# bkj/pytorch-graphsage

Measured on AMD Instinct MI355X. Metric: seed-nodes/sec, higher is better.
Workload: dtype bf16; 1 GPU; Reddit-shaped mean-aggregator 2-layer fanout 25/10 hidden 128/128 (BASELINE configs[1]); N=232965 D=602 nnz=98191232; batch_per_gpu=512, global_batch=512, rng=philox, engine=fused, launch=cmdlist, pipelined=False, batch_queue=True, parallelism=dp1, ranks=1

## Files before the change

include/gsage.h:

```cpp
#ifndef GSAGE_H
#define GSAGE_H

#include <stdint.h>

#ifdef __cplusplus
extern "C" {
#endif

#define GSAGE_ABI_VERSION 6

enum { GSAGE_F32 = 0, GSAGE_BF16 = 1, GSAGE_FP8 = 2 };
enum {
    GSAGE_OK = 0,
    GSAGE_EINVAL = -1,
    GSAGE_ELAUNCH = -2,
    GSAGE_ENODEV = -3
};
enum { GSAGE_POOL_MAX = 0, GSAGE_POOL_MEAN = 1 };
enum { GSAGE_ACT_NONE = 0, GSAGE_ACT_RELU = 1, GSAGE_ACT_TANH = 2 };

int gsage_abi_version(void);
const char *gsage_last_error(void);
uint64_t gsage_launch_count(void);
int gsage_debug_abort_trace(int fd);
// ... 83 lines not shown
int gsage_mt_choice_device(uint32_t *state, int64_t high, int64_t count, int32_t *out, void *stream);
int gsage_mt_choice_segments(uint32_t *state, int64_t high, int64_t n_seg, const int64_t *seg_off,
                             const int64_t *seg_cnt, int32_t *out, void *stream);

int gsage_mt_choice_par(uint32_t *state, int64_t high, int64_t n_seg, const int64_t *seg_cum, const int64_t *seg_off,
                        int64_t n_total, int32_t *out, const uint64_t *table, void *scratch, int64_t scratch_bytes,
                        int32_t n_wg, int32_t units_per_wg, void *stream);
int64_t gsage_mt_choice_par_scratch(int32_t n_wg);
int gsage_mt_jump_table(uint64_t *out, int64_t words);
int64_t gsage_mt_jump_table_words(void);
int gsage_mt_jump_host(const uint32_t *state, const uint64_t *poly, uint32_t *out);
void gsage_mt_permutation(void *mt, int64_t n, int64_t *out);

int gsage_gather_mean(const void *table, int dtype, int64_t ld, const int64_t *ids, int64_t M,
                      int32_t n, int64_t D, void *out, int out_dtype, int64_t out_ld,
                      void *stream);

int gsage_gather_mean_multi(int32_t n_seg, const void *const *tables, const int64_t *const *ids,
                            void *const *outs, const int64_t *M, const int32_t *n, int dtype,
                            int64_t ld, int64_t D, int out_dtype, int64_t out_ld, void *stream);

int gsage_quantize_fp8(const void *table, int dtype, int64_t ld, int64_t n_rows, int64_t D, void *table_q,
                       int64_t ld_q, float *scale, void *stream);

int gsage_gather_rows_fp8(const void *table_q, int64_t ld, const float *scale, const int64_t *ids, int64_t M,
                          int64_t D, void *out, int out_dtype, int64_t out_ld, void *stream);

int gsage_gather_mean_fp8(const void *table_q, int64_t ld, const float *scale, const int64_t *ids, int64_t M,
                          int32_t n, int64_t D, void *out, int out_dtype, int64_t out_ld, void *stream);
int gsage_gather_mean_multi_fp8(int32_t n_seg, const void *const *tables_q, const int64_t *const *ids,
                                void *const *outs, const int64_t *M, const int32_t *n, const float *scale,
                                int64_t ld, int64_t D, int out_dtype, int64_t out_ld, void *stream);

int gsage_segment_mean_bwd(const float *dagg, int64_t ld, int64_t M, int32_t n, int64_t D,
                           float *dneibs, int64_t out_ld, void *stream);

int gsage_scatter_add_rows(const float *rows, int64_t ld, const int64_t *ids, int64_t M,
                           int32_t n, int64_t D, float scale, float *table_grad,
                           int64_t table_ld, void *stream);

int gsage_linear_nt(const void *A, int dtype, int64_t lda, const int64_t *a_rows,
                    int a_rows_group0_only, const void *W, int64_t ldw, const float *bias,
                    void *C, int c_dtype, int64_t ldc, int64_t M, int64_t N, int64_t K, int act,
                    int groups, int64_t a_gstride, int64_t w_gstride, int64_t c_gstride,
                    void *stream);

int64_t gsage_packed_weight_elems(int64_t N, int64_t K, int32_t groups);
int gsage_pack_weight(const void *W, int dtype, int64_t ldw, int64_t w_gstride, int64_t N, int64_t K,
                      int32_t groups, void *Wp, void *stream);
int gsage_linear_nt_packed(const void *A, int64_t lda, const int64_t *a_rows, int a_rows_group0_only,
                           const void *Wp, const float *bias, void *C, int c_dtype, int64_t ldc,
                           int64_t M, int64_t N, int64_t K, int act, int groups, int64_t a_gstride,
                           int64_t c_gstride, void *stream);

int gsage_wgrad(const void *dC, int dtype, int64_t ldc, const void *A, int64_t lda, int64_t a_gstride, int64_t M,
                int64_t Ntot, int64_t K,
                int64_t n_per_group, int64_t rows_per_split, float *slabs, int64_t ldk, float *out,
                int64_t out_gstride, void *stream);
int gsage_wgrad_slabs(int64_t M, int64_t rows_per_split);
typedef struct gsage_wgrad_desc {
    const void *dC;
    const void *A;
    float *slabs;
    int64_t ldc, lda, a_gstride;
    int64_t M, Ntot, K, n_per_group, ldk, rows_per_split;
    const int64_t *a_rows;
} gsage_wgrad_desc;
int gsage_wgrad_multi(int32_t n_prob, const gsage_wgrad_desc *probs, int dtype, void *stream);
int gsage_wgrad_pair_ok(int dtype, int64_t M, int64_t Ntot, int64_t n_per_group, int64_t rows_per_split);
int gsage_wgrad_ticks_next(int64_t *tick, int64_t *tick1, int64_t inc1, int64_t *tick2, int64_t inc2);

int gsage_pool_mlp(const void *A, int dtype, int64_t lda, const int64_t *a_rows, const void *W,
                   int64_t ldw, const float *bias, int64_t M, int32_t n, int64_t H, int64_t K,
                   int pool, float *pooled, int64_t pooled_ld, int32_t *argmax, void *pooled_bf16,
                   int64_t pooled_bf16_ld, uint32_t *relu_mask, void *stream);

int gsage_pool_mlp_packed(const void *A, int64_t lda, const int64_t *a_rows, const void *Wp,
                          const float *bias, int64_t M, int32_t n, int64_t H, int64_t K, int pool,
                          float *pooled, int64_t pooled_ld, int32_t *argmax, void *pooled_bf16,
                          int64_t pooled_bf16_ld, uint32_t *relu_mask, void *stream);

int gsage_pool_route_bwd(const float *g, int64_t ldg, const float *pooled, int64_t ldp,
                         const int32_t *argmax, int64_t lda, int64_t M, int32_t n, int32_t H, void *out,
                         int out_dtype, int64_t ldo, void *stream);

int gsage_pool_route_mean_bwd(const float *g, int64_t ldg, const uint32_t *relu_mask, int64_t M, int32_t n,
                              int32_t H, void *out, int out_dtype, int64_t ldo, float *bias_part, int32_t n_part,
                              void *stream);

int gsage_pool_bias_partials(const float *g, int64_t ldg, const float *pooled, int64_t ldp, int64_t M,
                             int32_t H, float *part, int32_t n_part, void *stream);

int gsage_pool_merge_bwd(const void *Hprev, int dtype, int64_t ldh, const float *DX, int64_t ldx, int64_t r_x,
                         const float *DN, int64_t ldn, int64_t r0, void *dH, int64_t ldo, int64_t R,
                         int32_t D, void *stream);

int gsage_attn_aggregate(const float *na, int64_t na_ld, const float *xa, int64_t xa_ld,
                         const void *table, int dtype, int64_t ld, const int64_t *ids, int64_t M,
                         int32_t n, int64_t Ha, int64_t D, float *agg, int64_t agg_ld, float *ws,
                         void *stream);
int gsage_attn_aggregate_lp(const float *na, int64_t na_ld, const float *xa, int64_t xa_ld, const void *table,
                            int dtype, int64_t ld, const int64_t *ids, int64_t M, int32_t n, int64_t Ha, int64_t D,
                            float *agg, int64_t agg_ld, float *ws, void *agg_lp, int64_t agg_lp_ld, void *stream);
int gsage_attn_mlp2_fwd(const void *hid, int dtype, int64_t ldh, const void *W2, int64_t ldw, float *a, int64_t lda,
                        int64_t M, int32_t Ha, void *stream);
int gsage_attn_mlp2_bwd(const float *dan, int64_t ldn, const float *dax, int64_t ldx, const void *hid, int dtype,
// ... 249 lines not shown
```

pytorch-graphsage_amd/_native.py:

```python
import ctypes
import os

_HERE = os.path.dirname(os.path.abspath(__file__))
LIB_PATH = os.path.join(_HERE, "libgsage_hip.so")

F32, BF16, FP8 = 0, 1, 2
POOL_MAX, POOL_MEAN = 0, 1
ACT_NONE, ACT_RELU, ACT_TANH = 0, 1, 2
SEG_MEAN, SEG_MAX, SEG_SOFTMAX_WEIGHTED, SEG_WEIGHTED_MEAN = 0, 1, 2, 3
ABI_VERSION = 6

_vp = ctypes.c_void_p
_i64 = ctypes.c_int64
_i32 = ctypes.c_int32
_u32 = ctypes.c_uint32
_u64 = ctypes.c_uint64
_int = ctypes.c_int
_f32 = ctypes.c_float

SIGNATURES = {
    "gsage_abi_version": (_int, []),
    "gsage_last_error": (ctypes.c_char_p, []),
    "gsage_launch_count": (_u64, []),
    "gsage_debug_abort_trace": (_int, [_int]),
# ... 13 lines not shown
    "gsage_cmdlist_side_begin": (_int, []),
    "gsage_cmdlist_side_end": (_int, []),
    "gsage_cmdlist_join": (_int, []),
    "gsage_cmdlist_destroy": (None, [_vp]),
    "gsage_host_call": (_int, [_vp, _vp, _vp]),
    "gsage_comm_load": (_int, [ctypes.c_char_p]),
    "gsage_comm_unique_id": (_int, [_vp]),
    "gsage_comm_create": (_int, [_vp, _i32, _i32, ctypes.POINTER(_vp)]),
    "gsage_comm_destroy": (_int, [_vp]),
    "gsage_comm_all_reduce_f32": (_int, [_vp, _vp, _i64, _i32, _vp]),
    "gsage_comm_all_gather": (_int, [_vp, _vp, _vp, _i64, _vp]),
    "gsage_comm_group": (_int, [_vp, _i32, _vp]),
    "gsage_sort_rows_temp_bytes": (_i64, [_i64, _i32]),
    "gsage_sort_rows": (_int, [_vp, _i64, _i64, _i64, _i32, _vp, _vp, _vp, _i64, _vp]),
    "gsage_segment_sum_rows": (_int, [_vp, _vp, _i64, _vp, _i64, _i64, _vp, _i64, _i32, _f32, _vp, _i64, _vp]),
    "gsage_head_l1_sharded": (_int, [_vp, _i64, _vp, _vp, _vp, _i64, _i64, _i64, _vp, _vp, _int, _i64, _vp, _vp]),
    "gsage_sample_csr_sel": (_int, [_vp, _vp, _i64, _vp, _i64, _i32, _vp, _vp, _vp, _vp]),
    "gsage_sample_dense": (_int, [_vp, _i64, _i64, _vp, _i64, _vp, _i32, _vp, _vp, _vp]),
    "gsage_sample_csr_philox": (_int, [_vp, _vp, _i64, _vp, _i64, _i32, _u32, _u64, _vp, _u64, _u64,
                                       _vp, _vp, _vp, _vp]),
    "gsage_sample_hops_philox": (_int, [_vp, _vp, _i64, _vp, _i64, _i32, _vp, _u32, _u64, _vp, _u64, _u64,
                                        _vp, _vp, _i64, _vp, _vp]),
    "gsage_sample_hops": (_int, [_vp, _vp]),
    "gsage_counter_add": (_int, [_vp, _u64, _vp]),
    "gsage_copy_pair": (_int, [_vp, _vp, _i64, _vp, _vp, _i64, _vp]),
    "gsage_mt_create": (_vp, [_u32]),
    "gsage_mt_destroy": (None, [_vp]),
    "gsage_mt_seed": (None, [_vp, _u32]),
    "gsage_mt_choice_i32": (_i64, [_vp, _i64, _i64, _vp]),
    "gsage_mt_permutation": (None, [_vp, _i64, _vp]),
    "gsage_mt_choice_device": (_int, [_vp, _i64, _i64, _vp, _vp]),
    "gsage_mt_choice_segments": (_int, [_vp, _i64, _i64, _vp, _vp, _vp, _vp]),
    "gsage_mt_choice_par": (_int, [_vp, _i64, _i64, _vp, _vp, _i64, _vp, _vp, _vp, _i64, _i32, _i32, _vp]),
    "gsage_mt_choice_par_scratch": (_i64, [_i32]),
    "gsage_mt_jump_table": (_int, [_vp, _i64]),
    "gsage_mt_jump_table_words": (_i64, []),
    "gsage_mt_jump_host": (_int, [_vp, _vp, _vp]),
    "gsage_head_n_valid_next": (_int, [_vp]),
    "gsage_gather_role_next": (_int, [_vp]),
    "gsage_hops_role_next": (_int, [_vp]),
    "gsage_gather_mean": (_int, [_vp, _int, _i64, _vp, _i64, _i32, _i64, _vp, _int, _i64, _vp]),
    "gsage_gather_mean_multi": (_int, [_i32, _vp, _vp, _vp, _vp, _vp, _int, _i64, _i64, _int, _i64, _vp]),
    "gsage_gather_mean_multi_adam": (_int, [_i32, _vp, _vp, _vp, _vp, _vp, _int, _i64, _i64, _int, _i64,
                                            _vp, _vp, _vp]),
    "gsage_quantize_fp8": (_int, [_vp, _int, _i64, _i64, _i64, _vp, _i64, _vp, _vp]),
    "gsage_gather_rows_fp8": (_int, [_vp, _i64, _vp, _vp, _i64, _i64, _vp, _int, _i64, _vp]),
    "gsage_gather_mean_fp8": (_int, [_vp, _i64, _vp, _vp, _i64, _i32, _i64, _vp, _int, _i64, _vp]),
    "gsage_gather_mean_multi_fp8": (_int, [_i32, _vp, _vp, _vp, _vp, _vp, _vp, _i64, _i64, _int, _i64, _vp]),
    "gsage_segment_mean_bwd": (_int, [_vp, _i64, _i64, _i32, _i64, _vp, _i64, _vp]),
    "gsage_scatter_add_rows": (_int, [_vp, _i64, _vp, _i64, _i32, _i64, _f32, _vp, _i64, _vp]),
    "gsage_linear_nt": (_int, [_vp, _int, _i64, _vp, _int, _vp, _i64, _vp, _vp, _int, _i64, _i64,
                               _i64, _i64, _int, _int, _i64, _i64, _i64, _vp]),
    "gsage_packed_weight_elems": (_i64, [_i64, _i64, _i32]),
    "gsage_pack_weight": (_int, [_vp, _int, _i64, _i64, _i64, _i64, _i32, _vp, _vp]),
    "gsage_linear_nt_packed": (_int, [_vp, _i64, _vp, _int, _vp, _vp, _vp, _int, _i64, _i64, _i64, _i64, _int,
                                      _int, _i64, _i64, _vp]),
    "gsage_wgrad": (_int, [_vp, _int, _i64, _vp, _i64, _i64, _i64, _i64, _i64, _i64, _i64, _vp, _i64, _vp,
                           _i64, _vp]),
    "gsage_wgrad_slabs": (_int, [_i64, _i64]),
    "gsage_pool_route_bwd": (_int, [_vp, _i64, _vp, _i64, _vp, _i64, _i64, _i32, _i32, _vp, _int, _i64, _vp]),
    "gsage_wgrad_multi": (_int, [_i32, _vp, _int, _vp]),
    "gsage_wgrad_pair_ok": (_int, [_int, _i64, _i64, _i64, _i64]),
    "gsage_wgrad_ticks_next": (_int, [_vp, _vp, _i64, _vp, _i64]),
    "gsage_clip_adam_meet": (_int, [_vp, _vp]),
    "gsage_gather_adam_capacity": (_int, [_int, _i64]),
    "gsage_head_ce": (_int, [_vp, _i64, _vp, _vp, _vp, _i32, _i32, _i32, _vp, _vp, _int, _i64, _vp, _vp,
                             _vp, _vp, _vp, _i64, _vp]),
    "gsage_head_ce_scratch": (_i64, [_i32, _i32, _i32]),
    "gsage_mean_tail_ce": (_int, [_vp, _i32, _i32, _vp, _i64, _vp, _i64, _vp, _vp, _i32, _vp, _vp, _i64,
                                  _vp, _vp, _vp, _vp, _vp, _vp, _int, _vp]),
    "gsage_mean_tail_ce_scratch": (_i64, [_i32, _i32]),
    "gsage_mean_tail_mfma": (_int, [_vp, _i32, _i32, _vp, _i64, _vp, _i64, _vp, _vp, _i32, _vp, _vp, _i64,
                                    _vp, _vp, _vp, _vp, _vp, _vp, _vp]),
    "gsage_mean_tail_mfma_scratch": (_i64, [_i32, _i32]),
    "gsage_mean_tail_mfma_sampler_wgs": (_i32, [_i64, _i64]),
    "gsage_clip_adam_step": (_int, [_vp, _vp, _vp, _vp, _i64, _vp, _vp, _vp, _f32, _f32, _f32, _f32,
                                    _f32, _vp, _int, _i32, _vp, _i32, _vp, _i64, _vp, _i64, _vp]),
    "gsage_finalize_grads": (_int, [_vp, _i32, _i64, _vp, _vp, _vp, _vp, _i64, _vp, _i64, _vp]),
    "gsage_finalize_partials": (_int, [_i32, _i64]),
    "gsage_grad_sqnorm": (_int, [_vp, _i64, _vp, _i32, _vp]),
    "gsage_zero_rows": (_int, [_vp, _i64, _vp, _i64, _i64, _vp]),
    "gsage_colsum_partials": (_int, [_vp, _i64, _i64, _i32, _vp, _i32, _vp]),
    "gsage_rows_catch_up": (_int, [_vp, _vp, _i64, _vp, _i64, _i32, _vp]),
    "gsage_rows_catch_up_all": (_int, [_vp, _i32, _vp]),
    "gsage_rows_sqnorm": (_int, [_vp, _vp, _i64, _vp, _i64, _i32, _vp, _i32, _vp]),
    "gsage_rows_adam": (_int, [_vp, _vp, _i64, _vp, _i64, _i32, _vp, _i32, _vp]),
    "gsage_adam_partials": (_int, [_i64]),
    "gsage_prep_weights": (_int, [_vp, _i32, _i64, _vp, _i64, _vp, _i64, _vp]),
    "gsage_bwd_merge": (_int, [_vp, _int, _i64, _vp, _i64, _i64, _vp, _i64, _i64, _i64, _i32, _i32, _vp,
                               _vp, _vp]),
    "gsage_pool_mlp": (_int, [_vp, _int, _i64, _vp, _vp, _i64, _vp, _i64, _i32, _i64, _i64, _int,
                              _vp, _i64, _vp, _vp, _i64, _vp, _vp]),
    "gsage_pool_mlp_packed": (_int, [_vp, _i64, _vp, _vp, _vp, _i64, _i32, _i64, _i64, _int, _vp, _i64, _vp, _vp,
                                     _i64, _vp, _vp]),
    "gsage_pool_route_mean_bwd": (_int, [_vp, _i64, _vp, _i64, _i32, _i32, _vp, _int, _i64, _vp, _i32, _vp]),
    "gsage_pool_bias_partials": (_int, [_vp, _i64, _vp, _i64, _i64, _i32, _vp, _i32, _vp]),
    "gsage_pool_merge_bwd": (_int, [_vp, _int, _i64, _vp, _i64, _i64, _vp, _i64, _i64, _vp, _i64, _i64, _i32, _vp]),
    "gsage_attn_aggregate": (_int, [_vp, _i64, _vp, _i64, _vp, _int, _i64, _vp, _i64, _i32, _i64,
                                    _i64, _vp, _i64, _vp, _vp]),
    "gsage_attn_aggregate_lp": (_int, [_vp, _i64, _vp, _i64, _vp, _int, _i64, _vp, _i64, _i32, _i64,
                                       _i64, _vp, _i64, _vp, _vp, _i64, _vp]),
    "gsage_attn_fused_ok": (_int, [_int, _i64, _i64, _i32, _i64]),
    "gsage_attn_fused_fwd": (_int, [_vp, _int, _i64, _vp, _i64, _vp, _i64, _vp, _i64, _vp, _i64, _i64, _i32, _i64, _vp,
                                    _i64, _vp, _i64, _vp, _vp, _i64, _vp]),
    "gsage_attn_fused_bwd": (_int, [_vp, _int, _i64, _vp, _i64, _vp, _i64, _vp, _i64, _vp, _vp, _i64, _vp, _i64, _vp, _i64,
                                    _i64, _i32, _i64, _vp, _i64, _vp, _i64, _vp, _i64, _vp]),
# ... 253 lines not shown
```

pytorch-graphsage_amd/csrc/gsage_packed.hip:

```cpp
#include "gsage_common.h"
#include "gsage_gather_dev.h"
#include "gsage_mma_dev.h"
#include "gsage_sample_dev.h"

namespace gsage {

#ifndef GSAGE_WP_R
#define GSAGE_WP_R 4
#endif
constexpr int WP_R = GSAGE_WP_R;
constexpr int WP_WAIT = ((6 * (WP_R - 1)) & 15) | (7 << 4) | (15 << 8) | (((6 * (WP_R - 1)) >> 4) << 14);
static_assert(WP_R == 4 || WP_R == 6 || WP_R == 8, "WP_R");
static_assert(WP_R != 4 || WP_WAIT == 0x4F72, "vmcnt(18)");
constexpr int WP_NBUF = WP_R + 1;
constexpr int WP_UNROLL = 24;

struct PackedParams {
    const uint16_t *A;
    const uint16_t *Wp;
    const float *bias;
    const int64_t *a_rows;
    void *C;
    int64_t lda, ldc;
    int64_t M, N, K;
    int64_t a_gstride, wp_gstride, c_gstride;
    int32_t kc_total;
    int32_t a_rows_group0_only;
    int32_t c_dtype;
};

constexpr int WP_SMEM_VEC = (BM * (BN + 4) * 4) / 16 > WP_NBUF * (BM * CH) ? (BM * (BN + 4) * 4) / 16 : WP_NBUF * (BM * CH);

template <int ACT, int GN, bool HOPS>
__global__ void __launch_bounds__(256)
k_linear_nt_packed(const PackedParams p, const TailGather tg, const HopsParams hp)
{
    constexpr int EPC = 8;
    constexpr int ATILE = BM * CH;
    __shared__ vec16 smem[WP_SMEM_VEC];
    if (HOPS && blockIdx.z + 1 == gridDim.z) {
        sample_hops_workgroup<false>(hp, (int)(blockIdx.y * gridDim.x + blockIdx.x), reinterpret_cast<int64_t *>(smem));
        return;
    }
    if (GN > 0 && blockIdx.z + 1 == gridDim.z) {
        gather_role<(GN > 0 ? GN : 1), 2>(tg, (int)(blockIdx.y * gridDim.x + blockIdx.x));
        return;
    }

    const int tid = threadIdx.x;
    const int lane = tid & 63;
    const int wave = tid >> 6;
    const int g = blockIdx.z;
    const int64_t m0 = (int64_t)blockIdx.x * BM;
    const int64_t n0 = (int64_t)blockIdx.y * BN;
    const uint16_t *A = p.A + (int64_t)g * p.a_gstride;
    const int64_t *a_rows = (p.a_rows && (g == 0 || !p.a_rows_group0_only)) ? p.a_rows : nullptr;
    const int nk = (int)((p.K + 63) / 64);
    const int64_t jb_last = (p.N - 1) >> 5;
    const int64_t jb = min((n0 >> 5) + wave, jb_last);
    const vec16 *wp = reinterpret_cast<const vec16 *>(p.Wp + (int64_t)g * p.wp_gstride) +
                      (jb * p.kc_total) * 64 + lane;

    const int cdst = lane & 7;
    const uint16_t *a_src[2];
#pragma unroll
    for (int s2 = 0; s2 < 2; ++s2) {
        const int R = 32 * s2 + 8 * wave + (lane >> 3);
        const int row = (R & ~9) | ((R & 1) << 3) | ((R >> 3) & 1);
        int64_t m = m0 + row;
        if (m >= p.M) m = p.M - 1;
        const int64_t r = a_rows ? a_rows[m] : m;
        a_src[s2] = A + r * p.lda + (cdst ^ (row & 7)) * EPC;
    }
    const int a_dst0 = (8 * wave) * CH, a_dst1 = (32 + 8 * wave) * CH;

    vec16 wr[WP_R][4];
    auto issue_tile = [&](int kt, int buf, vec16 (&w)[4]) {
        vec16 *base = smem + buf * ATILE;
        const int64_t ko = (int64_t)kt * 64;
        __builtin_amdgcn_sched_barrier(0);
        __builtin_amdgcn_global_load_lds((global_void_t *)(a_src[0] + ko), (lds_void_t *)(base + a_dst0), 16, 0, 0);
        __builtin_amdgcn_global_load_lds((global_void_t *)(a_src[1] + ko), (lds_void_t *)(base + a_dst1), 16, 0, 0);
#pragma unroll
        for (int kk = 0; kk < 4; ++kk) w[kk] = wp[(int64_t)(kt * 4 + kk) * 64];
        __builtin_amdgcn_sched_barrier(0);
    };

    f32x16_t acc0, acc1;
#pragma unroll
    for (int r = 0; r < 16; ++r) { acc0[r] = 0.f; acc1[r] = 0.f; }
    const int arow0 = lane & 31, arow1 = arow0 + 32;

    auto compute_tile = [&](int kt, const vec16 (&w)[4]) {
        const vec16 *sA = smem + (kt % WP_NBUF) * ATILE;
        vec16 fa0[4], fa1[4];
#pragma unroll
        for (int kk = 0; kk < 4; ++kk) {
            const int ch = kk * 2 + (lane >> 5);
            fa0[kk] = sA[lds_slot(arow0, ch)];
            fa1[kk] = sA[lds_slot(arow1, ch)];
        }
        __builtin_amdgcn_s_waitcnt(0xC07F);
        __builtin_amdgcn_sched_barrier(0);
#pragma unroll
        for (int kk = 0; kk < 4; ++kk) {
            mma_chunk<uint16_t>::run(fa0[kk], w[kk], acc0);
            mma_chunk<uint16_t>::run(fa1[kk], w[kk], acc1);
        }
        __builtin_amdgcn_sched_barrier(0);
    };

    int kt = 0, phase = 0;
    if (nk > WP_R) {
#pragma unroll
        for (int t = 0; t < WP_R; ++t) issue_tile(t, t, wr[t]);
#pragma unroll
        for (int u = 0; u < WP_UNROLL; ++u) {
            if (kt + WP_R >= nk) { phase = u % WP_R; goto drain; }
            __builtin_amdgcn_s_waitcnt(WP_WAIT);
            __builtin_amdgcn_s_barrier();
            compute_tile(kt, wr[u % WP_R]);
            issue_tile(kt + WP_R, (kt + WP_R) % WP_NBUF, wr[u % WP_R]);
            ++kt;
        }
        for (;;) {
#pragma unroll
            for (int s = 0; s < WP_R; ++s) {
                if (kt + WP_R >= nk) { phase = s; goto drain; }
                __builtin_amdgcn_s_waitcnt(WP_WAIT);
                __builtin_amdgcn_s_barrier();
                compute_tile(kt, wr[s]);
                issue_tile(kt + WP_R, (kt + WP_R) % WP_NBUF, wr[s]);
                ++kt;
            }
        }
    } else {
#pragma unroll
        for (int t = 0; t < WP_R; ++t)
            if (t < nk) issue_tile(t, t, wr[t]);
    }
drain:
    __builtin_amdgcn_s_waitcnt(0x0F70);
    __builtin_amdgcn_s_barrier();
#pragma unroll
    for (int t = 0; t < WP_R; ++t) {
        if (kt + t < nk) {
            const int idx = (phase + t) % WP_R;
#pragma unroll
            for (int s = 0; s < WP_R; ++s)
                if (idx == s) compute_tile(kt + t, wr[s]);
        }
    }

    const float *bias = p.bias ? p.bias + (int64_t)g * p.N : nullptr;
    const int esz = p.c_dtype == GSAGE_BF16 ? 2 : 4;
    const int epc = 16 / esz;
    const int64_t cbase = (int64_t)g * p.c_gstride + n0;
    const bool wide = n0 + BN <= p.N && p.ldc % epc == 0 && cbase % epc == 0 && ((uintptr_t)p.C % 16) == 0;
    const int jl = wave * 32 + (lane & 31);
    const float bj = (bias && n0 + jl < p.N) ? bias[n0 + jl] : 0.f;
    if (wide) {
        __syncthreads();
        const int ldt = BN + epc;
#pragma unroll
        for (int rb = 0; rb < 2; ++rb) {
            const f32x16_t &acc = rb ? acc1 : acc0;
#pragma unroll
            for (int r = 0; r < 16; ++r) {
                const int i = rb * 32 + (r & 3) + 8 * (r >> 2) + 4 * (lane >> 5);
                const float v = apply_act(acc[r] + bj, ACT);
                if (p.c_dtype == GSAGE_BF16)
                    ((uint16_t *)smem)[i * ldt + jl] = f32_to_bf16(v);
                else
                    ((float *)smem)[i * ldt + jl] = v;
            }
        }
        __syncthreads();
        const int cpr = BN / epc;
        for (int q = tid; q < BM * cpr; q += 256) {
            const int row = q / cpr, ch = q - row * cpr;
            const int64_t m = m0 + row;
            if (m < p.M) {
                const vec16 v = *reinterpret_cast<const vec16 *>((const char *)smem +
                                                                 ((size_t)row * ldt + ch * epc) * esz);
                *reinterpret_cast<vec16 *>((char *)p.C + ((size_t)m * p.ldc + cbase + ch * epc) * esz) = v;
            }
        }
        return;
    }
    const int64_t j = n0 + jl;
#pragma unroll
    for (int rb = 0; rb < 2; ++rb) {
        const f32x16_t &acc = rb ? acc1 : acc0;
#pragma unroll
        for (int r = 0; r < 16; ++r) {
            const int64_t m = m0 + rb * 32 + (r & 3) + 8 * (r >> 2) + 4 * (lane >> 5);
            if (m < p.M && j < p.N) {
                const float v = apply_act(acc[r] + bj, ACT);
                const int64_t off = m * p.ldc + (int64_t)g * p.c_gstride + j;
                if (p.c_dtype == GSAGE_BF16)
                    ((uint16_t *)p.C)[off] = f32_to_bf16(v);
                else
                    ((float *)p.C)[off] = v;
            }
        }
    }
}

constexpr int WS_TPW = 8;
constexpr int WS_LDT = BN + 8;

template <int NK> constexpr int ws_ring() { return NK == 3 ? 3 : 4; }
template <int NK> constexpr size_t ws_lds_bytes()
{
    return (size_t)(ws_ring<NK>() + 1) * BM * CH * 16 + (size_t)BM * WS_LDT * 2 + (size_t)WS_TPW * 2 * 256 * 4;
}

template <int N>
__device__ __forceinline__ void ws_wait_vm()
{
    static_assert(N >= 0 && N < 64, "vmcnt is six bits");
    asm volatile("s_waitcnt vmcnt(%0)" ::"n"(N) : "memory");
}

template <int BASE, int STEP>
__device__ __forceinline__ void ws_wait_vm_sel(int t)
{
    if (t == 0) ws_wait_vm<BASE>();
    else if (t == 1) ws_wait_vm<BASE + STEP>();
    else if (t == 2) ws_wait_vm<BASE + 2 * STEP>();
    else ws_wait_vm<BASE + 3 * STEP>();
}

template <int ACT, int NK>
__global__ void __launch_bounds__(256)
k_linear_nt_packed_ws(const PackedParams p, const int tpw)
{
    constexpr int R = ws_ring<NK>(), TR = R / NK, NBUF = R + 1, ATILE = BM * CH, NST = 4;
    constexpr int STEADY = 2 * (R - 1) + NST * TR;
    extern __shared__ __attribute__((aligned(16))) char ws_smem[];
    vec16 *ring = reinterpret_cast<vec16 *>(ws_smem);
    uint16_t *stage = reinterpret_cast<uint16_t *>(ws_smem + (size_t)NBUF * ATILE * 16);
    uint32_t *rid_s = reinterpret_cast<uint32_t *>(ws_smem + (size_t)NBUF * ATILE * 16 + (size_t)BM * WS_LDT * 2);

    const int tid = threadIdx.x, lane = tid & 63;
    const int wave = __builtin_amdgcn_readfirstlane(tid >> 6);
    const int g = blockIdx.z;
    const int64_t n0 = (int64_t)blockIdx.y * BN;
    const int64_t n_tiles = (p.M + BM - 1) / BM;
    const int64_t tile0 = (int64_t)blockIdx.x * tpw;
    const uint16_t *A = p.A + (int64_t)g * p.a_gstride;
// ... 389 lines not shown
                sum += v;
                if (v > best) { best = v; arg = r; }
            }
            if (p.pool_mode == GSAGE_POOL_MAX) {
                p.pooled[seg * p.pooled_ld + j] = best;
                if (p.pooled_b) p.pooled_b[seg * p.pooled_b_ld + j] = f32_to_bf16(best);
                if (p.argmax) p.argmax[seg * p.N + j] = arg;
            } else {
                p.pooled[seg * p.pooled_ld + j] = sum / (float)p.pool_n;
                if (p.pooled_b) p.pooled_b[seg * p.pooled_b_ld + j] = f32_to_bf16(sum / (float)p.pool_n);
            }
        }
    }
}


template <typename TW>
__global__ void __launch_bounds__(256)
k_pack_weight(const TW *__restrict__ W, int64_t ldw, int64_t w_gstride, int64_t N, int64_t K,
              int32_t kc_total, int32_t jb_total, int32_t groups, uint16_t *__restrict__ Wp)
{
    const int64_t total = (int64_t)groups * jb_total * kc_total * 64;
    const int64_t stride = (int64_t)gridDim.x * 256;
    for (int64_t t = (int64_t)blockIdx.x * 256 + threadIdx.x; t < total; t += stride) {
        const int lane = (int)(t & 63);
        int64_t u = t >> 6;
        const int kc = (int)(u % kc_total);
        u /= kc_total;
        const int jb = (int)(u % jb_total);
        const int g = (int)(u / jb_total);
        const int64_t j = (int64_t)jb * 32 + (lane & 31);
        const int64_t k0 = (int64_t)kc * 16 + (lane >> 5) * 8;
        uint16_t out[8];
#pragma unroll
        for (int e = 0; e < 8; ++e) {
            float v = 0.f;
            if (j < N && k0 + e < K) {
                const TW w = W[(int64_t)g * w_gstride + j * ldw + k0 + e];
                v = sizeof(TW) == 2 ? bf16_to_f32((uint16_t)w) : (float)w;
            }
            out[e] = f32_to_bf16(v);
        }
        vec16 o;
#pragma unroll
        for (int e = 0; e < 4; ++e) o[e] = (uint32_t)out[2 * e] | ((uint32_t)out[2 * e + 1] << 16);
        reinterpret_cast<vec16 *>(Wp)[t] = o;
    }
}

}

using namespace gsage;

extern "C" {

int64_t gsage_packed_weight_elems(int64_t N, int64_t K, int32_t groups)
{
    return (int64_t)groups * ceil_div(N, 32) * (ceil_div(K, 64) * 4) * 64 * 8;
}

int gsage_pack_weight(const void *W, int dtype, int64_t ldw, int64_t w_gstride, int64_t N, int64_t K,
                      int32_t groups, void *Wp, void *stream)
{
    GSAGE_REQUIRE(W && Wp && N > 0 && K > 0 && groups >= 1 && ldw >= K, "pack_weight: bad arguments");
    GSAGE_REQUIRE(dtype == GSAGE_BF16 || dtype == GSAGE_F32, "pack_weight: bad dtype %d", dtype);
    GSAGE_REQUIRE(((uintptr_t)Wp % 16) == 0, "pack_weight: output must be 16-byte aligned");
    const int32_t kc = (int32_t)(ceil_div(K, 64) * 4), jb = (int32_t)ceil_div(N, 32);
    const int64_t slots = (int64_t)groups * jb * kc * 64;
    int64_t blocks = ceil_div(slots, 256);
    if (blocks > 4096) blocks = 4096;
    if (dtype == GSAGE_BF16)
        launch(k_pack_weight<uint16_t>, dim3((unsigned)blocks), dim3(256), 0, (hipStream_t)stream,
               (const uint16_t *)W, ldw, w_gstride, N, K, kc, jb, groups, (uint16_t *)Wp);
    else
        launch(k_pack_weight<float>, dim3((unsigned)blocks), dim3(256), 0, (hipStream_t)stream,
               (const float *)W, ldw, w_gstride, N, K, kc, jb, groups, (uint16_t *)Wp);
    return check_launch("pack_weight");
}

int gsage_linear_nt_packed(const void *A, int64_t lda, const int64_t *a_rows, int a_rows_group0_only,
                           const void *Wp, const float *bias, void *C, int c_dtype, int64_t ldc,
                           int64_t M, int64_t N, int64_t K, int act, int groups, int64_t a_gstride,
                           int64_t c_gstride, void *stream)
{
    const gsage_tail_gather_desc *gd = take_gather_role();
    const gsage_hops_desc *hd = t_hops_role;
    t_hops_role = nullptr;
    GSAGE_REQUIRE(A && Wp && C, "linear_nt_packed: null pointer");
    GSAGE_REQUIRE(M >= 0 && N > 0 && K > 0, "linear_nt_packed: bad sizes");
    GSAGE_REQUIRE(c_dtype == GSAGE_BF16 || c_dtype == GSAGE_F32, "linear_nt_packed: bad c_dtype");
    GSAGE_REQUIRE(groups >= 1 && groups <= 65535, "linear_nt_packed: bad group count");
    GSAGE_REQUIRE(act >= ACT_NONE && act <= ACT_TANH, "linear_nt_packed: bad activation code");
    GSAGE_REQUIRE(lda % 64 == 0 && ceil_div(K, 64) * 64 <= lda && ((uintptr_t)A % 16) == 0 &&
                  ((uintptr_t)Wp % 16) == 0, "linear_nt_packed: A rows must be whole zero-padded 128-byte lines");
    if (M == 0) return GSAGE_OK;
    PackedParams p;
    p.A = (const uint16_t *)A; p.Wp = (const uint16_t *)Wp; p.bias = bias; p.a_rows = a_rows; p.C = C;
    p.lda = lda; p.ldc = ldc; p.M = M; p.N = N; p.K = K;
    p.a_gstride = a_gstride; p.c_gstride = c_gstride;
    p.kc_total = (int32_t)(ceil_div(K, 64) * 4);
    p.wp_gstride = ceil_div(N, 32) * (int64_t)p.kc_total * 64 * 8;
    p.a_rows_group0_only = a_rows_group0_only; p.c_dtype = c_dtype;
    dim3 grid((unsigned)ceil_div(M, BM), (unsigned)ceil_div(N, BN), (unsigned)groups);
    hipStream_t s = (hipStream_t)stream;
    TailGather tg = {};
    HopsParams hp = {};
    if (hd) {
        GSAGE_REQUIRE(!(gd && gd->rows > 0) && act == ACT_RELU && !hd->dense_adj,
                      "linear_nt_packed: the sampler role rides with the ReLU projection, walks a CSR, and excludes the "
                      "gather role");
        size_t lds = 0;
        const int rc = fill_hops(hp, lds, *hd);
        if (rc != GSAGE_OK) return rc;
        const int64_t slots = (int64_t)grid.x * grid.y;
        hp.spw = (int32_t)ceil_div(hd->B > 0 ? hd->B : 1, slots);
        int64_t widest = 1, width = 1;
        for (int k = 1; k <= hp.n_hops; ++k) { width *= hp.fan[k]; widest = width > widest ? width : widest; }
        GSAGE_REQUIRE(sizeof(int64_t) * 2 * (size_t)hp.spw * (size_t)widest <= sizeof(vec16) * WP_SMEM_VEC,
                      "linear_nt_packed: the sampler role's frontier (%d seeds x %lld ids, twice) does not fit the "
                      "projection's LDS", hp.spw, (long long)widest);
        grid.z += 1;
        launch(k_linear_nt_packed<ACT_RELU, 0, true>, grid, dim3(256), 0, s, p, tg, hp);
        return check_launch("linear_nt_packed");
    }
    if (gd && gd->rows > 0) {
        const int rc = fill_gather_role(tg, *gd, "linear_nt_packed (gather role)");
        if (rc != GSAGE_OK) return rc;
        GSAGE_REQUIRE(act == ACT_RELU && (gd->n == 10 || gd->n == 5),
                      "linear_nt_packed: the gather role rides with the ReLU projection, fan-out 5 or 10");
        tg.n_wg = (int32_t)(grid.x * grid.y);
        grid.z += 1;
        if (gd->n == 10) launch(k_linear_nt_packed<ACT_RELU, 10, false>, grid, dim3(256), 0, s, p, tg, hp);
        else launch(k_linear_nt_packed<ACT_RELU, 5, false>, grid, dim3(256), 0, s, p, tg, hp);
        return check_launch("linear_nt_packed");
    }
    {
        const char *ws_env = getenv("GSAGE_K5_WS");
        const bool ws_on = !ws_env || atoi(ws_env) != 0;
        const int nk = (int)ceil_div(K, 64);
        const int tr = nk == 1 ? 4 : nk == 2 ? 2 : 1;
        const int64_t n_tiles = ceil_div(M, BM);
        if (ws_on && c_dtype == GSAGE_BF16 && nk <= 4 && N % BN == 0 && ldc % 8 == 0 && c_gstride % 8 == 0 &&
            ((uintptr_t)C % 16) == 0 && n_tiles >= 4 * tr && (act == ACT_RELU || act == ACT_NONE)) {
            int dev = 0, cus = 256;
            if (hipGetDevice(&dev) == hipSuccess) {
                int v = 0;
                if (hipDeviceGetAttribute(&v, hipDeviceAttributeMultiprocessorCount, dev) == hipSuccess && v > 0) cus = v;
                else (void)hipGetLastError();
            } else (void)hipGetLastError();
            const int64_t slices = (int64_t)grid.y * groups;
            int64_t per = ceil_div(2 * (int64_t)cus, slices);
            if (per < 1) per = 1;
            int64_t tpw = ceil_div(n_tiles, per);
            if (const char *e = getenv("GSAGE_K5_WS_TPW")) tpw = atoi(e);
            if (tpw < tr) tpw = tr;
            if (tpw > WS_TPW) tpw = WS_TPW;
            grid.x = (unsigned)ceil_div(n_tiles, tpw);
#define GSAGE_WS_LAUNCH(ACTV, NKV)                                                                                        \
            do {                                                                                                      \
                static bool raised = false;                                                                           \
                if (!raised) {                                                                                        \
                    if (hipFuncSetAttribute((const void *)k_linear_nt_packed_ws<ACTV, NKV>,                           \
                                            hipFuncAttributeMaxDynamicSharedMemorySize, (int)ws_lds_bytes<NKV>()) != hipSuccess) { \
                        (void)hipGetLastError();                                                                      \
                        set_error("linear_nt_packed: cannot raise the dynamic LDS limit");                          \
                        return GSAGE_ELAUNCH;                                                                         \
                    }                                                                                                 \
                    raised = true;                                                                                    \
                }                                                                                                     \
                launch(k_linear_nt_packed_ws<ACTV, NKV>, grid, dim3(256), ws_lds_bytes<NKV>(), s, p, (int)tpw);       \
            } while (0)
#define GSAGE_WS_NK(ACTV)                                                                                                 \
            do {                                                                                                      \
                if (nk == 1) GSAGE_WS_LAUNCH(ACTV, 1);                                                                \
                else if (nk == 2) GSAGE_WS_LAUNCH(ACTV, 2);                                                           \
                else if (nk == 3) GSAGE_WS_LAUNCH(ACTV, 3);                                                           \
                else GSAGE_WS_LAUNCH(ACTV, 4);                                                                        \
            } while (0)
            if (act == ACT_RELU) GSAGE_WS_NK(ACT_RELU);
            else GSAGE_WS_NK(ACT_NONE);
#undef GSAGE_WS_NK
#undef GSAGE_WS_LAUNCH
            return check_launch("linear_nt_packed");
        }
    }
    if (act == ACT_RELU)
        launch(k_linear_nt_packed<ACT_RELU, 0, false>, grid, dim3(256), 0, s, p, tg, hp);
    else if (act == ACT_TANH)
        launch(k_linear_nt_packed<ACT_TANH, 0, false>, grid, dim3(256), 0, s, p, tg, hp);
    else
        launch(k_linear_nt_packed<ACT_NONE, 0, false>, grid, dim3(256), 0, s, p, tg, hp);
    return check_launch("linear_nt_packed");
}

int gsage_pool_mlp_packed(const void *A, int64_t lda, const int64_t *a_rows, const void *Wp,
                          const float *bias, int64_t M, int32_t n, int64_t H, int64_t K, int pool,
                          float *pooled, int64_t pooled_ld, int32_t *argmax, void *pooled_bf16,
                          int64_t pooled_bf16_ld, uint32_t *relu_mask, void *stream)
{
    GSAGE_REQUIRE(A && Wp && pooled && pooled_ld >= H, "pool_mlp_packed: bad pointers / output");
    GSAGE_REQUIRE(M >= 0 && H > 0 && K > 0, "pool_mlp_packed: bad sizes");
    GSAGE_REQUIRE(n >= 1 && n <= BM, "pool_mlp_packed: fanout must be in [1, %d]", BM);
    GSAGE_REQUIRE(!relu_mask || H % 32 == 0, "pool_mlp_packed: relu_mask needs H % 32 == 0");
    GSAGE_REQUIRE(!pooled_bf16 || pooled_bf16_ld >= H, "pool_mlp_packed: bad bf16 output");
    GSAGE_REQUIRE(pool == GSAGE_POOL_MAX || pool == GSAGE_POOL_MEAN, "pool_mlp_packed: bad pool mode");
    GSAGE_REQUIRE(lda % 64 == 0 && ceil_div(K, 64) * 64 <= lda && ((uintptr_t)A % 16) == 0 &&
                  ((uintptr_t)Wp % 16) == 0, "pool_mlp_packed: A rows must be whole zero-padded 128-byte lines");
    if (M == 0) return GSAGE_OK;
    PoolPackedParams p;
    p.A = (const uint16_t *)A; p.Wp = (const uint16_t *)Wp; p.bias = bias; p.a_rows = a_rows; p.lda = lda;
    p.M = M * (int64_t)n; p.N = H; p.K = K; p.kc_total = (int32_t)(ceil_div(K, 64) * 4);
    p.pool_n = n; p.pool_groups = BM / n; p.pool_mode = pool; p.pooled = pooled; p.pooled_ld = pooled_ld;
    p.pooled_b = (uint16_t *)pooled_bf16; p.pooled_b_ld = pooled_bf16_ld; p.argmax = argmax;
    p.relu_mask = relu_mask;
    const int64_t subs = ceil_div(M, p.pool_groups);
    dim3 grid((unsigned)subs, (unsigned)ceil_div(H, 256), 1);
    static const bool regs = [] { const char *e = getenv("GSAGE_POOL_REGS"); return !e || atoi(e) != 0; }();
    const bool rp = regs && pool == GSAGE_POOL_MAX && !relu_mask;
    hipStream_t s = (hipStream_t)stream;
    if (rp && n == 10) launch(k_pool_mlp_packed<4, 10>, grid, dim3(256), 0, s, p);
    else if (rp && n == 25) launch(k_pool_mlp_packed<4, 25>, grid, dim3(256), 0, s, p);
    else if (rp && n == 5) launch(k_pool_mlp_packed<4, 5>, grid, dim3(256), 0, s, p);
    else if (rp && n == 15) launch(k_pool_mlp_packed<4, 15>, grid, dim3(256), 0, s, p);
    else if (rp && n == 20) launch(k_pool_mlp_packed<4, 20>, grid, dim3(256), 0, s, p);
    else launch(k_pool_mlp_packed<4, 0>, grid, dim3(256), 0, s, p);
    return check_launch("pool_mlp_packed");
}

}
```

Measured before the change: 6.368 million seed-nodes/sec.

## Add tall 128-row tile variant to packed projection kernel when grid oversubscribes CUs

```diff
diff --git a/include/gsage.h b/include/gsage.h
--- a/include/gsage.h
+++ b/include/gsage.h
@@ -159,6 +159,7 @@
                            const void *Wp, const float *bias, void *C, int c_dtype, int64_t ldc,
                            int64_t M, int64_t N, int64_t K, int act, int groups, int64_t a_gstride,
                            int64_t c_gstride, void *stream);
+int gsage_packed_last_rows(void);
 
 int gsage_wgrad(const void *dC, int dtype, int64_t ldc, const void *A, int64_t lda, int64_t a_gstride, int64_t M,
                 int64_t Ntot, int64_t K,
diff --git a/pytorch-graphsage_amd/_native.py b/pytorch-graphsage_amd/_native.py
--- a/pytorch-graphsage_amd/_native.py
+++ b/pytorch-graphsage_amd/_native.py
@@ -89,6 +89,7 @@
     "gsage_linear_nt": (_int, [_vp, _int, _i64, _vp, _int, _vp, _i64, _vp, _vp, _int, _i64, _i64,
                                _i64, _i64, _int, _int, _i64, _i64, _i64, _vp]),
     "gsage_packed_weight_elems": (_i64, [_i64, _i64, _i32]),
+    "gsage_packed_last_rows": (_int, []),
     "gsage_pack_weight": (_int, [_vp, _int, _i64, _i64, _i64, _i64, _i32, _vp, _vp]),
     "gsage_linear_nt_packed": (_int, [_vp, _i64, _vp, _int, _vp, _vp, _vp, _int, _i64, _i64, _i64, _i64, _int,
                                       _int, _i64, _i64, _vp]),
diff --git a/pytorch-graphsage_amd/csrc/gsage_packed.hip b/pytorch-graphsage_amd/csrc/gsage_packed.hip
--- a/pytorch-graphsage_amd/csrc/gsage_packed.hip
+++ b/pytorch-graphsage_amd/csrc/gsage_packed.hip
@@ -8,11 +8,23 @@
 #ifndef GSAGE_WP_R
 #define GSAGE_WP_R 4
 #endif
+#ifndef GSAGE_WP_RT
+#define GSAGE_WP_RT 4
+#endif
 constexpr int WP_R = GSAGE_WP_R;
-constexpr int WP_WAIT = ((6 * (WP_R - 1)) & 15) | (7 << 4) | (15 << 8) | (((6 * (WP_R - 1)) >> 4) << 14);
+constexpr int WP_BMT = 128;
+constexpr int WP_RT = GSAGE_WP_RT;
+constexpr int wp_tile_vm(int bmt) { return bmt / 32 + 4; }
+constexpr int wp_wait(int bmt, int r)
+{
+    return ((wp_tile_vm(bmt) * (r - 1)) & 15) | (7 << 4) | (15 << 8) | (((wp_tile_vm(bmt) * (r - 1)) >> 4) << 14);
+}
 static_assert(WP_R == 4 || WP_R == 6 || WP_R == 8, "WP_R");
-static_assert(WP_R != 4 || WP_WAIT == 0x4F72, "vmcnt(18)");
-constexpr int WP_NBUF = WP_R + 1;
+static_assert(WP_RT == 4 || WP_RT == 6, "WP_RT");
+static_assert(wp_tile_vm(WP_BMT) * (WP_RT - 1) < 64 && wp_tile_vm(BM) * (WP_R - 1) < 64, "vmcnt is six bits");
+static_assert(WP_R != 4 || wp_wait(BM, WP_R) == 0x4F72, "vmcnt(18)");
+static_assert(wp_wait(WP_BMT, 4) == 0x4F78, "vmcnt(24)");
+static_assert(wp_wait(WP_BMT, 6) == 0x8F78, "vmcnt(40)");
 constexpr int WP_UNROLL = 24;
 
 struct PackedParams {
@@ -29,15 +41,30 @@
     int32_t c_dtype;
 };
 
-constexpr int WP_SMEM_VEC = (BM * (BN + 4) * 4) / 16 > WP_NBUF * (BM * CH) ? (BM * (BN + 4) * 4) / 16 : WP_NBUF * (BM * CH);
-
-template <int ACT, int GN, bool HOPS>
+constexpr int wp_smem_vec(int bmt, int r)
+{
+    return (bmt * (BN + 4) * 4) / 16 > (r + 1) * (bmt * CH) ? (bmt * (BN + 4) * 4) / 16 : (r + 1) * (bmt * CH);
+}
+
+template <int ACT, int GN, bool HOPS, int BMT = BM, int R = WP_R>
 __global__ void __launch_bounds__(256)
 k_linear_nt_packed(const PackedParams p, const TailGather tg, const HopsParams hp)
 {
     constexpr int EPC = 8;
-    constexpr int ATILE = BM * CH;
-    __shared__ vec16 smem[WP_SMEM_VEC];
+    constexpr int NRB = BMT / 32;
+    constexpr int NBUF = R + 1;
+    constexpr int WAIT = wp_wait(BMT, R);
+    constexpr int ATILE = BMT * CH;
+    static_assert(BMT == BM || BMT == WP_BMT, "BMT");
+    static_assert(WP_UNROLL % R == 0, "WP_UNROLL");
+    vec16 *smem;
+    if constexpr (BMT == BM) {
+        __shared__ vec16 smem_static[wp_smem_vec(BMT, R)];
+        smem = smem_static;
+    } else {
+        extern __shared__ __attribute__((aligned(16))) vec16 smem_tall[];
+        smem = smem_tall;
+    }
     if (HOPS && blockIdx.z + 1 == gridDim.z) {
         sample_hops_workgroup<false>(hp, (int)(blockIdx.y * gridDim.x + blockIdx.x), reinterpret_cast<int64_t *>(smem));
         return;
@@ -51,7 +78,7 @@
     const int lane = tid & 63;
     const int wave = tid >> 6;
     const int g = blockIdx.z;
-    const int64_t m0 = (int64_t)blockIdx.x * BM;
+    const int64_t m0 = (int64_t)blockIdx.x * BMT;
     const int64_t n0 = (int64_t)blockIdx.y * BN;
     const uint16_t *A = p.A + (int64_t)g * p.a_gstride;
     const int64_t *a_rows = (p.a_rows && (g == 0 || !p.a_rows_group0_only)) ? p.a_rows : nullptr;
@@ -62,92 +89,96 @@
                       (jb * p.kc_total) * 64 + lane;
 
     const int cdst = lane & 7;
-    const uint16_t *a_src[2];
-#pragma unroll
-    for (int s2 = 0; s2 < 2; ++s2) {
-        const int R = 32 * s2 + 8 * wave + (lane >> 3);
-        const int row = (R & ~9) | ((R & 1) << 3) | ((R >> 3) & 1);
+    const uint16_t *a_src[NRB];
+#pragma unroll
+    for (int s2 = 0; s2 < NRB; ++s2) {
+        const int R0 = 32 * s2 + 8 * wave + (lane >> 3);
+        const int row = (R0 & ~9) | ((R0 & 1) << 3) | ((R0 >> 3) & 1);
         int64_t m = m0 + row;
         if (m >= p.M) m = p.M - 1;
         const int64_t r = a_rows ? a_rows[m] : m;
         a_src[s2] = A + r * p.lda + (cdst ^ (row & 7)) * EPC;
     }
-    const int a_dst0 = (8 * wave) * CH, a_dst1 = (32 + 8 * wave) * CH;
-
-    vec16 wr[WP_R][4];
+    const int a_dst0 = (8 * wave) * CH;
+
+    vec16 wr[R][4];
     auto issue_tile = [&](int kt, int buf, vec16 (&w)[4]) {
         vec16 *base = smem + buf * ATILE;
         const int64_t ko = (int64_t)kt * 64;
         __builtin_amdgcn_sched_barrier(0);
-        __builtin_amdgcn_global_load_lds((global_void_t *)(a_src[0] + ko), (lds_void_t *)(base + a_dst0), 16, 0, 0);
-        __builtin_amdgcn_global_load_lds((global_void_t *)(a_src[1] + ko), (lds_void_t *)(base + a_dst1), 16, 0, 0);
+#pragma unroll
+        for (int s2 = 0; s2 < NRB; ++s2)
+            __builtin_amdgcn_global_load_lds((global_void_t *)(a_src[s2] + ko),
+                                             (lds_void_t *)(base + a_dst0 + s2 * 32 * CH), 16, 0, 0);
 #pragma unroll
         for (int kk = 0; kk < 4; ++kk) w[kk] = wp[(int64_t)(kt * 4 + kk) * 64];
         __builtin_amdgcn_sched_barrier(0);
     };
 
-    f32x16_t acc0, acc1;
-#pragma unroll
-    for (int r = 0; r < 16; ++r) { acc0[r] = 0.f; acc1[r] = 0.f; }
-    const int arow0 = lane & 31, arow1 = arow0 + 32;
+    f32x16_t acc[NRB];
+#pragma unroll
+    for (int rb = 0; rb < NRB; ++rb)
+#pragma unroll
+        for (int r = 0; r < 16; ++r) acc[rb][r] = 0.f;
+    const int arow0 = lane & 31;
 
     auto compute_tile = [&](int kt, const vec16 (&w)[4]) {
-        const vec16 *sA = smem + (kt % WP_NBUF) * ATILE;
-        vec16 fa0[4], fa1[4];
+        const vec16 *sA = smem + (kt % NBUF) * ATILE;
+        vec16 fa[NRB][4];
 #pragma unroll
         for (int kk = 0; kk < 4; ++kk) {
             const int ch = kk * 2 + (lane >> 5);
-            fa0[kk] = sA[lds_slot(arow0, ch)];
-            fa1[kk] = sA[lds_slot(arow1, ch)];
+#pragma unroll
+            for (int rb = 0; rb < NRB; ++rb) fa[rb][kk] = sA[lds_slot(arow0 + 32 * rb, ch)];
         }
         __builtin_amdgcn_s_waitcnt(0xC07F);
         __builtin_amdgcn_sched_barrier(0);
 #pragma unroll
         for (int kk = 0; kk < 4; ++kk) {
-            mma_chunk<uint16_t>::run(fa0[kk], w[kk], acc0);
-            mma_chunk<uint16_t>::run(fa1[kk], w[kk], acc1);
+#pragma unroll
+            for (int rb = 0; rb < NRB; ++rb) mma_chunk<uint16_t>::run(fa[rb][kk], w[kk], acc[rb]);
         }
         __builtin_amdgcn_sched_barrier(0);
     };
 
     int kt = 0, phase = 0;
-    if (nk > WP_R) {
-#pragma unroll
-        for (int t = 0; t < WP_R; ++t) issue_tile(t, t, wr[t]);
+    if (nk > R) {
+#pragma unroll
+        for (int t = 0; t < R; ++t) issue_tile(t, t, wr[t]);
 #pragma unroll
         for (int u = 0; u < WP_UNROLL; ++u) {
-            if (kt + WP_R >= nk) { phase = u % WP_R; goto drain; }
-            __builtin_amdgcn_s_waitcnt(WP_WAIT);
+            if (kt + R >= nk) { phase = u % R; goto drain; }
+            __builtin_amdgcn_s_waitcnt(WAIT);
             __builtin_amdgcn_s_barrier();
-            compute_tile(kt, wr[u % WP_R]);
-            issue_tile(kt + WP_R, (kt + WP_R) % WP_NBUF, wr[u % WP_R]);
+            compute_tile(kt, wr[u % R]);
+            issue_tile(kt + R, (kt + R) % NBUF, wr[u % R]);
             ++kt;
         }
         for (;;) {
 #pragma unroll
-            for (int s = 0; s < WP_R; ++s) {
-                if (kt + WP_R >= nk) { phase = s; goto drain; }
-                __builtin_amdgcn_s_waitcnt(WP_WAIT);
+            for (int s = 0; s < R; ++s) {
+                if (kt + R >= nk) { phase = s; goto drain; }
+                __builtin_amdgcn_s_waitcnt(WAIT);
                 __builtin_amdgcn_s_barrier();
                 compute_tile(kt, wr[s]);
-                issue_tile(kt + WP_R, (kt + WP_R) % WP_NBUF, wr[s]);
+                issue_tile(kt + R, (kt + R) % NBUF, wr[s]);
                 ++kt;
             }
         }
     } else {
 #pragma unroll
-        for (int t = 0; t < WP_R; ++t)
+        for (int t = 0; t < R; ++t)
             if (t < nk) issue_tile(t, t, wr[t]);
     }
 drain:
     __builtin_amdgcn_s_waitcnt(0x0F70);
     __builtin_amdgcn_s_barrier();
 #pragma unroll
-    for (int t = 0; t < WP_R; ++t) {
+    for (int t = 0; t < R; ++t) {
         if (kt + t < nk) {
-            const int idx = (phase + t) % WP_R;
-#pragma unroll
-            for (int s = 0; s < WP_R; ++s)
+            const int idx = (phase + t) % R;
+#pragma unroll
+            for (int s = 0; s < R; ++s)
                 if (idx == s) compute_tile(kt + t, wr[s]);
         }
     }
@@ -163,12 +194,11 @@
         __syncthreads();
         const int ldt = BN + epc;
 #pragma unroll
-        for (int rb = 0; rb < 2; ++rb) {
-            const f32x16_t &acc = rb ? acc1 : acc0;
+        for (int rb = 0; rb < NRB; ++rb) {
 #pragma unroll
             for (int r = 0; r < 16; ++r) {
                 const int i = rb * 32 + (r & 3) + 8 * (r >> 2) + 4 * (lane >> 5);
-                const float v = apply_act(acc[r] + bj, ACT);
+                const float v = apply_act(acc[rb][r] + bj, ACT);
                 if (p.c_dtype == GSAGE_BF16)
                     ((uint16_t *)smem)[i * ldt + jl] = f32_to_bf16(v);
                 else
@@ -177,7 +207,7 @@
         }
         __syncthreads();
         const int cpr = BN / epc;
-        for (int q = tid; q < BM * cpr; q += 256) {
+        for (int q = tid; q < BMT * cpr; q += 256) {
             const int row = q / cpr, ch = q - row * cpr;
             const int64_t m = m0 + row;
             if (m < p.M) {
@@ -190,13 +220,12 @@
     }
     const int64_t j = n0 + jl;
 #pragma unroll
-    for (int rb = 0; rb < 2; ++rb) {
-        const f32x16_t &acc = rb ? acc1 : acc0;
+    for (int rb = 0; rb < NRB; ++rb) {
 #pragma unroll
         for (int r = 0; r < 16; ++r) {
             const int64_t m = m0 + rb * 32 + (r & 3) + 8 * (r >> 2) + 4 * (lane >> 5);
             if (m < p.M && j < p.N) {
-                const float v = apply_act(acc[r] + bj, ACT);
+                const float v = apply_act(acc[rb][r] + bj, ACT);
                 const int64_t off = m * p.ldc + (int64_t)g * p.c_gstride + j;
                 if (p.c_dtype == GSAGE_BF16)
                     ((uint16_t *)p.C)[off] = f32_to_bf16(v);
@@ -692,7 +721,64 @@
 
 using namespace gsage;
 
+namespace {
+
+constexpr size_t WP_TALL_LDS = sizeof(vec16) * wp_smem_vec(WP_BMT, WP_RT);
+constexpr int WP_MAX_DEV = 64;
+
+thread_local int t_last_rows = 0;
+
+int current_cus(int &dev)
+{
+    int cus = 256;
+    dev = 0;
+    if (hipGetDevice(&dev) == hipSuccess) {
+        int v = 0;
+        if (hipDeviceGetAttribute(&v, hipDeviceAttributeMultiprocessorCount, dev) == hipSuccess && v > 0) cus = v;
+        else (void)hipGetLastError();
+    } else (void)hipGetLastError();
+    return cus;
+}
+
+bool wants_tall_tiles(int64_t M, int64_t N, int groups, int cus)
+{
+    const char *e = getenv("GSAGE_K5_BM");
+    const int forced = e ? atoi(e) : 0;
+    if (M < WP_BMT || forced == BM) return false;
+    if (forced == WP_BMT) return true;
+    return ceil_div(M, BM) * ceil_div(N, BN) * groups > cus;
+}
+
+template <int ACT, int GN, bool HOPS>
+bool tall_tiles_ok(int dev)
+{
+    static std::atomic<int> state[WP_MAX_DEV];
+    if (dev < 0 || dev >= WP_MAX_DEV) return false;
+    int st = state[dev].load(std::memory_order_acquire);
+    if (st == 0) {
+        st = hipFuncSetAttribute((const void *)k_linear_nt_packed<ACT, GN, HOPS, WP_BMT, WP_RT>,
+                                 hipFuncAttributeMaxDynamicSharedMemorySize, (int)WP_TALL_LDS) == hipSuccess ? 1 : -1;
+        if (st < 0) (void)hipGetLastError();
+        state[dev].store(st, std::memory_order_release);
+    }
+    return st > 0;
+}
+
+template <int ACT, int GN, bool HOPS>
+void launch_k5(bool tall, dim3 grid, hipStream_t s, const PackedParams &p, const TailGather &tg, const HopsParams &hp)
+{
+    t_last_rows = tall ? WP_BMT : BM;
+    if (tall)
+        launch(k_linear_nt_packed<ACT, GN, HOPS, WP_BMT, WP_RT>, grid, dim3(256), WP_TALL_LDS, s, p, tg, hp);
+    else
+        launch(k_linear_nt_packed<ACT, GN, HOPS>, grid, dim3(256), 0, s, p, tg, hp);
+}
+
+}
+
 extern "C" {
+
+int gsage_packed_last_rows(void) { return t_last_rows; }
 
 int64_t gsage_packed_weight_elems(int64_t N, int64_t K, int32_t groups)
 {
@@ -743,6 +829,9 @@
     p.a_rows_group0_only = a_rows_group0_only; p.c_dtype = c_dtype;
     dim3 grid((unsigned)ceil_div(M, BM), (unsigned)ceil_div(N, BN), (unsigned)groups);
     hipStream_t s = (hipStream_t)stream;
+    int dev = 0;
+    const int cus = current_cus(dev);
+    bool tall = wants_tall_tiles(M, N, groups, cus);
     TailGather tg = {};
     HopsParams hp = {};
     if (hd) {
@@ -752,15 +841,18 @@
         size_t lds = 0;
         const int rc = fill_hops(hp, lds, *hd);
         if (rc != GSAGE_OK) return rc;
+        tall = tall && tall_tiles_ok<ACT_RELU, 0, true>(dev);
+        if (tall) grid.x = (unsigned)ceil_div(M, WP_BMT);
         const int64_t slots = (int64_t)grid.x * grid.y;
         hp.spw = (int32_t)ceil_div(hd->B > 0 ? hd->B : 1, slots);
         int64_t widest = 1, width = 1;
         for (int k = 1; k <= hp.n_hops; ++k) { width *= hp.fan[k]; widest = width > widest ? width : widest; }
-        GSAGE_REQUIRE(sizeof(int64_t) * 2 * (size_t)hp.spw * (size_t)widest <= sizeof(vec16) * WP_SMEM_VEC,
+        GSAGE_REQUIRE(sizeof(int64_t) * 2 * (size_t)hp.spw * (size_t)widest <=
+                          (tall ? WP_TALL_LDS : sizeof(vec16) * wp_smem_vec(BM, WP_R)),
                       "linear_nt_packed: the sampler role's frontier (%d seeds x %lld ids, twice) does not fit the "
                       "projection's LDS", hp.spw, (long long)widest);
         grid.z += 1;
-        launch(k_linear_nt_packed<ACT_RELU, 0, true>, grid, dim3(256), 0, s, p, tg, hp);
+        launch_k5<ACT_RELU, 0, true>(tall, grid, s, p, tg, hp);
         return check_launch("linear_nt_packed");
     }
     if (gd && gd->rows > 0) {
@@ -768,10 +860,12 @@
         if (rc != GSAGE_OK) return rc;
         GSAGE_REQUIRE(act == ACT_RELU && (gd->n == 10 || gd->n == 5),
                       "linear_nt_packed: the gather role rides with the ReLU projection, fan-out 5 or 10");
+        tall = tall && (gd->n == 10 ? tall_tiles_ok<ACT_RELU, 10, false>(dev) : tall_tiles_ok<ACT_RELU, 5, false>(dev));
+        if (tall) grid.x = (unsigned)ceil_div(M, WP_BMT);
         tg.n_wg = (int32_t)(grid.x * grid.y);
         grid.z += 1;
-        if (gd->n == 10) launch(k_linear_nt_packed<ACT_RELU, 10, false>, grid, dim3(256), 0, s, p, tg, hp);
-        else launch(k_linear_nt_packed<ACT_RELU, 5, false>, grid, dim3(256), 0, s, p, tg, hp);
+        if (gd->n == 10) launch_k5<ACT_RELU, 10, false>(tall, grid, s, p, tg, hp);
+        else launch_k5<ACT_RELU, 5, false>(tall, grid, s, p, tg, hp);
         return check_launch("linear_nt_packed");
     }
     {
@@ -782,12 +876,6 @@
         const int64_t n_tiles = ceil_div(M, BM);
         if (ws_on && c_dtype == GSAGE_BF16 && nk <= 4 && N % BN == 0 && ldc % 8 == 0 && c_gstride % 8 == 0 &&
             ((uintptr_t)C % 16) == 0 && n_tiles >= 4 * tr && (act == ACT_RELU || act == ACT_NONE)) {
-            int dev = 0, cus = 256;
-            if (hipGetDevice(&dev) == hipSuccess) {
-                int v = 0;
-                if (hipDeviceGetAttribute(&v, hipDeviceAttributeMultiprocessorCount, dev) == hipSuccess && v > 0) cus = v;
-                else (void)hipGetLastError();
-            } else (void)hipGetLastError();
             const int64_t slices = (int64_t)grid.y * groups;
             int64_t per = ceil_div(2 * (int64_t)cus, slices);
             if (per < 1) per = 1;
@@ -817,6 +905,7 @@
                 else if (nk == 3) GSAGE_WS_LAUNCH(ACTV, 3);                                                           \
                 else GSAGE_WS_LAUNCH(ACTV, 4);                                                                        \
             } while (0)
+            t_last_rows = 0;
             if (act == ACT_RELU) GSAGE_WS_NK(ACT_RELU);
             else GSAGE_WS_NK(ACT_NONE);
 #undef GSAGE_WS_NK
@@ -824,12 +913,12 @@
             return check_launch("linear_nt_packed");
         }
     }
-    if (act == ACT_RELU)
-        launch(k_linear_nt_packed<ACT_RELU, 0, false>, grid, dim3(256), 0, s, p, tg, hp);
-    else if (act == ACT_TANH)
-        launch(k_linear_nt_packed<ACT_TANH, 0, false>, grid, dim3(256), 0, s, p, tg, hp);
-    else
-        launch(k_linear_nt_packed<ACT_NONE, 0, false>, grid, dim3(256), 0, s, p, tg, hp);
+    tall = tall && (act == ACT_RELU ? tall_tiles_ok<ACT_RELU, 0, false>(dev)
+                    : act == ACT_TANH ? tall_tiles_ok<ACT_TANH, 0, false>(dev) : tall_tiles_ok<ACT_NONE, 0, false>(dev));
+    if (tall) grid.x = (unsigned)ceil_div(M, WP_BMT);
+    if (act == ACT_RELU) launch_k5<ACT_RELU, 0, false>(tall, grid, s, p, tg, hp);
+    else if (act == ACT_TANH) launch_k5<ACT_TANH, 0, false>(tall, grid, s, p, tg, hp);
+    else launch_k5<ACT_NONE, 0, false>(tall, grid, s, p, tg, hp);
     return check_launch("linear_nt_packed");
 }
 
```

New measurement: 6.130 million seed-nodes/sec. -3.7%, worse.
